# breuner/elbencho

Hardware: AMD Instinct MI355X
Metric: seq-read GiB/s into GPU HBM (higher is better)
Workload: dtype raw-bytes; 1 GPU; seqread; model=storage-benchmark seq-read into HBM, threads_per_gpu=16, block_size=4194304, iodepth=1, bench_dir=/dev/shm/elbencho_amd_bench, gpu_staged=True, mmap_zero_copy=True, dynamic_slice=True, verify_on_gpu=True, verify_salt=7, parallelism=single, device=AMD Radeon Graphics, device_numa_node=0

## Files before the change

elbencho_amd/csrc/engine.cpp:

```cpp

#include "engine.h"

#include <fcntl.h>
#include <linux/fs.h>
#include <pthread.h>
#include <sched.h>
#include <sys/ioctl.h>
#include <sys/mman.h>
#include <sys/stat.h>
#include <sys/types.h>
#include <unistd.h>

#include <algorithm>
#include <random>
#include <cerrno>
#include <cstdio>
#include <cstring>

#include "netbench.h"
#include "uring.h"

namespace eb {

static constexpr uint64_t INTERRUPT_CHECK_INTERVAL = 128;
// ... 898 lines not shown

    const uint64_t mapBPF = (cfg.random || cfg.strided) ? (fileSize / bs) : numBlocksPerFile;
    const uint64_t virtFileLen = mapBPF * bs;

    const bool dynamic = cfg.dynamicSlice && !cfg.random && !cfg.strided &&
                         !cfg.backward && cfg.numThreads == cfg.numDataSetThreads;

    std::unique_ptr<OffsetGen> gen;
    if (dynamic) {
    } else if (cfg.random || cfg.strided) {
        uint64_t numBlocksTotal = mapBPF * numFiles;
        uint64_t rangeLen = bs * (numBlocksTotal / cfg.numDataSetThreads);
        uint64_t rangeOff = (uint64_t)globalRank * rangeLen;
        if (cfg.strided) {
            gen = std::make_unique<OffsetGenStrided>(bs, globalRank, cfg.numDataSetThreads);
            gen->reset(0, bs * numBlocksTotal);
        } else {
            gen = makeOffsetGen(rangeOff, rangeLen);
        }
    } else {
        uint64_t myStart, myLen;
        fairShareSlice(virtFileLen * numFiles, myStart, myLen);
        if (!myLen) return;
        gen = makeOffsetGen(myStart, myLen);
    }

    const int nSlots = (int)hostBufs.size();
    constexpr uint64_t VERIFY_FETCH_INTERVAL = 64;
    uint64_t sinceFetch = 0;
    BlockSpec spec;
    uint64_t opCount = 0;
    int slot = 0;

    auto fetchVerify = [&]() {
        GpuVerifyResult r = gpu->fetchVerifyResult();
        if (r.numMismatches)
            throw WorkerError("Data verification failed (GPU). First bad file offset: " +
                              std::to_string(r.firstBadFileOffset) +
                              "; mismatching 8-byte words: " +
                              std::to_string(r.numMismatches));
    };

    if (doVerify && !isWrite) (void)gpu->fetchVerifyResult();

    const uint64_t totalBlocks = numBlocksPerFile * numFiles;

    auto nextBlock = [&](uint64_t& fileIdx, uint64_t& inFileOff,
                         uint64_t& ioLen) -> bool {
        if (dynamic) {
            for (;;) {
                uint64_t b = eng.dynCursor.fetch_add(1, std::memory_order_relaxed);
                if (b >= totalBlocks) return false;
                fileIdx = b / numBlocksPerFile;
                inFileOff = (b % numBlocksPerFile) * bs;
                if (inFileOff >= fileSize) continue;
                ioLen = std::min(bs, fileSize - inFileOff);
                return true;
            }
        }
        while (gen->next(spec)) {
            if (!virtFileLen) return false;
            fileIdx = spec.offset / virtFileLen;
            if (fileIdx >= numFiles) continue;
            inFileOff = spec.offset - fileIdx * virtFileLen;
            if (inFileOff >= fileSize) continue;
            ioLen = std::min(spec.len, fileSize - inFileOff);
            return true;
        }
        return false;
    };

    uint64_t fileIdx, inFileOff, ioLen;
    while (nextBlock(fileIdx, inFileOff, ioLen)) {
        if ((opCount++ % INTERRUPT_CHECK_INTERVAL) == 0) checkInterrupt();

        rateLimiter.wait(ioLen);

        if (lat && gpu->timedPairActive(slot))
            addIoLat(gpu->timedElapsedUSec(slot));

        if (isWrite) {
            preWriteFill(slot, ioLen, inFileOff);
            if (lat) gpu->recordTimedStart(slot);
            gpu->copyToHostAsync(slot, bases[fileIdx] + inFileOff, ioLen);
            if (lat) gpu->recordTimedEnd(slot);
        } else {
            if (lat) gpu->recordTimedStart(slot);
            gpu->copyFromHostAsync(slot, bases[fileIdx] + inFileOff, ioLen);
            if (lat) gpu->recordTimedEnd(slot);
            if (doVerify && (inFileOff % 8 == 0) && (ioLen % 16 == 0)) {
                gpu->verifyChecksumDevAsync(slot, ioLen, inFileOff,
                                            (uint64_t)cfg.verifySalt);
                if (++sinceFetch >= VERIFY_FETCH_INTERVAL) {
                    fetchVerify();
                    sinceFetch = 0;
                }
            } else if (doVerify) {
                uint64_t bad = verifyChecksumCPU(bases[fileIdx] + inFileOff, ioLen,
                                                 inFileOff, (uint64_t)cfg.verifySalt);
                if (bad != UINT64_MAX)
                    throw WorkerError("Data verification failed. First bad file offset: " +
                                      std::to_string(bad));
            }
        }

        liveOps.bytes.fetch_add(ioLen, std::memory_order_relaxed);
        liveOps.iops.fetch_add(1, std::memory_order_relaxed);
        slot = (slot + 1) % nSlots;

        if ((opCount & 127) == 0) gpu->syncStream();
    }

    gpu->syncStream();
    if (lat)
        for (int s = 0; s < nSlots; s++)
            if (gpu->timedPairActive(s)) addIoLat(gpu->timedElapsedUSec(s));
    if (doVerify && !isWrite) fetchVerify();
}

void Worker::fileModeBlocksUring(bool isWrite)
{
    const auto& cfg = eng.cfg;
    const uint64_t fileSize = eng.effFileSize;
    const uint64_t bs = cfg.blockSize;
    const size_t numFiles = cfg.paths.size();
    const uint64_t numBlocksPerFile = (fileSize + bs - 1) / bs;
    const int depth = cfg.ioDepth;
    const bool lat = cfg.measureLat;

    const bool rwMixActive = isWrite && (cfg.rwMixPct > 0 || isDedicatedReader);

    FdGuard fg;
    int rwFlags = isWrite ? ((cfg.verifyDirect || rwMixActive) ? O_RDWR : O_WRONLY) : O_RDONLY;
    int openFlags = rwFlags | (cfg.directIO ? O_DIRECT : 0);
    if (isWrite && cfg.pathType == PathType::FILE) openFlags |= O_CREAT;
    for (const auto& p : cfg.paths) {
        int fd = open(p.c_str(), openFlags, 0644);
        if (fd < 0) throwErrno("open", p);
        fg.fds.push_back(fd);
        if (isWrite && cfg.pathType == PathType::FILE) {
            if (cfg.truncate && ftruncate(fd, 0)) throwErrno("truncate", p);
            if (cfg.truncToSize != UINT64_MAX && ftruncate(fd, fileSize))
                throwErrno("truncate-to-size", p);
            if (cfg.preallocFile && fallocate(fd, 0, 0, fileSize)) throwErrno("fallocate", p);
        }
        applyFadvise(fd, cfg.fadviseFlags, p);
    }

    const uint64_t mapBPF = (cfg.random || cfg.strided) ? (fileSize / bs) : numBlocksPerFile;
    const uint64_t virtFileLen = mapBPF * bs;
// ... 1858 lines not shown
```

elbencho_amd/csrc/gpu.h:

```cpp

#pragma once

#include <cstdint>
#include <string>
#include <vector>

#include "crc.h"

namespace eb {

struct GpuVerifyResult {
    uint64_t numMismatches;
    uint64_t firstBadFileOffset;
};

void gpuHostRegister(void* ptr, uint64_t len);
bool gpuHostRegisterTry(void* ptr, uint64_t len);
void gpuHostUnregister(void* ptr);

class GpuCtx;

int gpuDeviceCount();

double gpuVerifyBenchGBs(uint64_t len, int iters, bool lds, int dev);

uint64_t gpuCrcTileBytes();
uint64_t gpuCrcWaveBytes();

std::string gpuProbeError();

std::string gpuDeviceName(int deviceId);

int gpuNumaNode(int deviceId);

class GpuCtx {
public:
    GpuCtx(int deviceId, int numSlots, uint64_t bufSize, bool pinnedHostBufs);
    ~GpuCtx();
    GpuCtx(const GpuCtx&) = delete;
    GpuCtx& operator=(const GpuCtx&) = delete;

    int deviceId() const { return devId; }
    char* hostBuf(int slot) const;
    uint64_t bufSize() const { return slotSize; }
    int numSlots() const { return slots; }
    uint64_t slotStride() const;

    void snapshotSlots(std::vector<char>& dst);

    void bindThread();

    void copyFromHostAsync(int slot, const void* src, uint64_t len);
    void copyToHostAsync(int slot, void* dst, uint64_t len);
    void copyH2DAsync(int slot, uint64_t len);
    void copyH2DRangeAsync(int firstSlot, int count);
    void copyD2HAsync(int slot, uint64_t len);
    void syncStream();

    void recordSlotEvent(int slot);
    void waitSlotEvent(int slot);

    void recordTimedStart(int slot);
    void recordTimedEnd(int slot);
    bool timedPairActive(int slot) const;
    uint64_t timedElapsedUSec(int slot);

    void verifyChecksumDevAsync(int slot, uint64_t len, uint64_t fileOff, uint64_t salt,
                                bool ldsVariant = false);
    GpuVerifyResult fetchVerifyResult();


    void fillRandDev(int slot, uint64_t len, uint64_t seed, bool fastAlgo = false);

    void fillChecksumDev(int slot, uint64_t len, uint64_t fileOff, uint64_t salt);

    GpuVerifyResult verifyChecksumDev(int slot, uint64_t len, uint64_t fileOff, uint64_t salt,
                                      bool ldsVariant = false);

    void blockVarRefillDev(int slot, uint64_t len, uint64_t refillLen, uint64_t seed,
                           bool fastAlgo = false);


    void crcDevAsync(int slot, uint64_t len, CrcAlgo algo, uint64_t partialBase);

    uint32_t crcFetch(CrcAlgo algo, uint64_t totalLen, uint64_t tileCount);

    uint32_t crcDev(int slot, uint64_t len, CrcAlgo algo);

private:
    struct Impl;
    Impl* impl;
    int devId;
    uint64_t slotSize;
    int slots;
};

}
```

elbencho_amd/csrc/gpu_kernels.hip:

```cpp

#include <hip/hip_runtime.h>

#include <cstdio>
#include <map>
#include <mutex>
#include <stdexcept>
#include <string>
#include <vector>

#include "crc.h"
#include "gpu.h"

namespace eb {

#define HIP_CHECK(cmd)                                                                 \
    do {                                                                               \
        hipError_t e = (cmd);                                                          \
        if (e != hipSuccess)                                                           \
            throw std::runtime_error(std::string("HIP error: ") + hipGetErrorString(e) \
                                     + " at " __FILE__ ":" + std::to_string(__LINE__)); \
    } while (0)


__device__ __forceinline__ uint64_t d_splitmix64(uint64_t& state)
{
    uint64_t z = (state += 0x9E3779B97F4A7C15ULL);
    z = (z ^ (z >> 30)) * 0xBF58476D1CE4E5B9ULL;
    z = (z ^ (z >> 27)) * 0x94D049BB133111EBULL;
    return z ^ (z >> 31);
}

__device__ __forceinline__ uint64_t d_rotl64(uint64_t x, int k)
{
    return (x << k) | (x >> (64 - k));
}
// ... 141 lines not shown
        uint64_t exp0 = off0 + salt;
        uint64_t exp1 = off0 + 8 + salt;
        if (v.x != exp0) {
            localBad++;
            if (off0 < localFirst) localFirst = off0;
        }
        if (v.y != exp1) {
            localBad++;
            if (off0 + 8 < localFirst) localFirst = off0 + 8;
        }
    }

    if (tid == 0 && (n64 & 1)) {
        uint64_t offT = fileOff + (n64 - 1) * 8;
        if (((const uint64_t*)buf)[n64 - 1] != offT + salt) {
            localBad++;
            if (offT < localFirst) localFirst = offT;
        }
    }

#pragma unroll
    for (int delta = 32; delta > 0; delta >>= 1) {
        localBad += __shfl_down(localBad, delta, 64);
        unsigned long long other = __shfl_down(localFirst, delta, 64);
        if (other < localFirst) localFirst = other;
    }

    if ((threadIdx.x & 63) == 0 && localBad) {
        atomicAdd(&out[0], localBad);
        atomicMin(&out[1], localFirst);
    }
}

__global__ __launch_bounds__(256) void ebVerifyChecksumLdsKernel(
    const ulonglong2* __restrict__ buf, uint64_t n64, uint64_t fileOff,
    uint64_t salt, unsigned long long* __restrict__ out)
{
    const uint64_t nVec2 = n64 / 2;
    constexpr int VPT = 4;
    __shared__ ulonglong2 lds[256 * VPT];
    __shared__ unsigned long long blkBad, blkFirst;
    if (threadIdx.x == 0) {
        blkBad = 0;
        blkFirst = ~0ULL;
    }
    __syncthreads();

    unsigned long long localBad = 0, localFirst = ~0ULL;
    const uint64_t tileElems = (uint64_t)blockDim.x * VPT;

    for (uint64_t tileBase = (uint64_t)blockIdx.x * tileElems; tileBase < nVec2;
         tileBase += (uint64_t)gridDim.x * tileElems) {
#pragma unroll
        for (int v = 0; v < VPT; v++) {
            uint64_t idx = tileBase + (uint64_t)v * blockDim.x + threadIdx.x;
            if (idx < nVec2) lds[v * blockDim.x + threadIdx.x] = buf[idx];
        }
        __syncthreads();
#pragma unroll
        for (int v = 0; v < VPT; v++) {
            uint64_t idx = tileBase + (uint64_t)v * blockDim.x + threadIdx.x;
            if (idx >= nVec2) continue;
            ulonglong2 val = lds[v * blockDim.x + threadIdx.x];
            uint64_t off0 = fileOff + idx * 16;
            if (val.x != off0 + salt) {
                localBad++;
// ... 201 lines not shown
static hipStream_t sharedStream(int devId, int& poolSizeOut)
{
    static std::mutex mtx;
    static std::map<int, std::vector<hipStream_t>> pools;
    static std::map<int, int> next;
    static const int poolSize = [] {
        const char* v = getenv("EB_GPU_SHARED_STREAMS");
        int n = v ? atoi(v) : 8;
        return (n >= 1 && n <= 64) ? n : 0;
    }();

    poolSizeOut = poolSize;
    if (!poolSize) return nullptr;

    std::lock_guard<std::mutex> lk(mtx);
    auto& pool = pools[devId];
    if (pool.empty()) {
        pool.resize(poolSize);
        for (int i = 0; i < poolSize; i++)
            HIP_CHECK(hipStreamCreateWithFlags(&pool[i], hipStreamNonBlocking));
    }
    return pool[next[devId]++ % poolSize];
}

struct GpuCtx::Impl {
    hipStream_t stream = nullptr;
    bool ownStream = true;
    char* devBase = nullptr;
    char* hostBase = nullptr;
    uint64_t slotStride = 0;
    std::vector<char*> devBufs;
    std::vector<char*> hostBufs;
    std::vector<hipEvent_t> slotEvents;
    std::vector<hipEvent_t> timedStart, timedEnd;
    std::vector<char> timedActive;
    bool hostPinned = false;
    unsigned long long* verifyOutDev = nullptr;
    unsigned long long* verifyOutHost = nullptr;
    uint64_t fillCallCounter = 0;
    bool verifyDirty = false;

    uint32_t* crcTabDev[2] = {nullptr, nullptr};
    CrcShift crcTileShift[2];
    uint32_t* crcPartDev = nullptr;
    uint32_t* crcPartHost = nullptr;
    uint64_t crcPartCap = 0;
    struct CrcCall { uint64_t base, len; };
    std::vector<CrcCall> crcPending;
};

GpuCtx::GpuCtx(int deviceId, int numSlots, uint64_t bufSize, bool pinnedHostBufs)
    : impl(new Impl), devId(deviceId), slotSize(bufSize), slots(numSlots)
{
    HIP_CHECK(hipSetDevice(deviceId));
    int poolSize = 0;
    hipStream_t shared = sharedStream(deviceId, poolSize);
    if (shared) {
        impl->stream = shared;
        impl->ownStream = false;
    } else {
        HIP_CHECK(hipStreamCreateWithFlags(&impl->stream, hipStreamNonBlocking));
    }

    impl->hostPinned = pinnedHostBufs;
    impl->devBufs.resize(numSlots, nullptr);
    impl->hostBufs.resize(numSlots, nullptr);

    impl->slotStride = (bufSize + 4095) & ~4095ULL;
    HIP_CHECK(hipMalloc(&impl->devBase, impl->slotStride * numSlots));
    if (pinnedHostBufs) {
        static const unsigned hostFlags = [] {
            const char* v = getenv("EB_GPU_HOSTALLOC");
            return (v && v[0] == 'n') ? hipHostMallocNonCoherent : hipHostMallocDefault;
        }();
        HIP_CHECK(hipHostMalloc(&impl->hostBase, impl->slotStride * numSlots, hostFlags));
    } else {
        if (posix_memalign((void**)&impl->hostBase, 4096, impl->slotStride * numSlots))
            throw std::runtime_error("host buffer alloc failed");
    }
    for (int i = 0; i < numSlots; i++) {
        impl->devBufs[i] = impl->devBase + (uint64_t)i * impl->slotStride;
        impl->hostBufs[i] = impl->hostBase + (uint64_t)i * impl->slotStride;
    }

    impl->slotEvents.resize(numSlots, nullptr);
    static const bool evBlock = [] {
        const char* v = getenv("EB_GPU_EVBLOCK");
        return v && v[0] == '1';
    }();
    unsigned evFlags = hipEventDisableTiming | (evBlock ? hipEventBlockingSync : 0);
    for (int i = 0; i < numSlots; i++)
        HIP_CHECK(hipEventCreateWithFlags(&impl->slotEvents[i], evFlags));

    HIP_CHECK(hipMalloc(&impl->verifyOutDev, 2 * sizeof(unsigned long long)));
    HIP_CHECK(hipHostMalloc(&impl->verifyOutHost, 2 * sizeof(unsigned long long),
                            hipHostMallocDefault));

    impl->verifyOutHost[0] = 0;
    impl->verifyOutHost[1] = ~0ULL;
    HIP_CHECK(hipMemcpy(impl->verifyOutDev, impl->verifyOutHost,
                        2 * sizeof(unsigned long long), hipMemcpyHostToDevice));
}

GpuCtx::~GpuCtx()
{
    (void)hipSetDevice(devId);
    if (impl->devBase) (void)hipFree(impl->devBase);
    if (impl->hostBase) {
        if (impl->hostPinned)
            (void)hipHostFree(impl->hostBase);
        else
            free(impl->hostBase);
    }
    for (auto e : impl->slotEvents)
        if (e) (void)hipEventDestroy(e);
    for (auto e : impl->timedStart)
        if (e) (void)hipEventDestroy(e);
    for (auto e : impl->timedEnd)
        if (e) (void)hipEventDestroy(e);
    if (impl->verifyOutDev) (void)hipFree(impl->verifyOutDev);
    if (impl->verifyOutHost) (void)hipHostFree(impl->verifyOutHost);
    for (auto p : impl->crcTabDev)
        if (p) (void)hipFree(p);
    if (impl->crcPartDev) (void)hipFree(impl->crcPartDev);
    if (impl->crcPartHost) (void)hipHostFree(impl->crcPartHost);
    if (impl->stream && impl->ownStream) (void)hipStreamDestroy(impl->stream);
    delete impl;
}

char* GpuCtx::hostBuf(int slot) const { return impl->hostBufs[slot]; }

void GpuCtx::bindThread() { HIP_CHECK(hipSetDevice(devId)); }

uint64_t GpuCtx::slotStride() const { return impl->slotStride; }

void GpuCtx::snapshotSlots(std::vector<char>& dst)
{
    dst.resize(impl->slotStride * (uint64_t)slots);
    if (dst.empty()) return;
    HIP_CHECK(hipMemcpyAsync(dst.data(), impl->devBase, dst.size(), hipMemcpyDeviceToHost,
                             impl->stream));
    HIP_CHECK(hipStreamSynchronize(impl->stream));
}

void GpuCtx::copyFromHostAsync(int slot, const void* src, uint64_t len)
{
    HIP_CHECK(hipMemcpyAsync(impl->devBufs[slot], src, len, hipMemcpyHostToDevice,
                             impl->stream));
}

void GpuCtx::copyToHostAsync(int slot, void* dst, uint64_t len)
{
    HIP_CHECK(hipMemcpyAsync(dst, impl->devBufs[slot], len, hipMemcpyDeviceToHost,
                             impl->stream));
// ... 65 lines not shown
    return (uint64_t)(ms * 1000.0f);
}

static void requireAligned(const char* what, uint64_t len, uint64_t lenAlign,
                           uint64_t fileOff = 0)
{
    if (len % lenAlign)
        throw std::invalid_argument(std::string(what) + ": len " + std::to_string(len) +
                                    " is not a multiple of " + std::to_string(lenAlign));
    if (fileOff % 8)
        throw std::invalid_argument(std::string(what) + ": fileOff " +
                                    std::to_string(fileOff) + " is not a multiple of 8");
}

void GpuCtx::verifyChecksumDevAsync(int slot, uint64_t len, uint64_t fileOff, uint64_t salt,
                                    bool ldsVariant)
{
    requireAligned("verifyChecksumDev", len, 8, fileOff);
    uint64_t n64 = len / 8;
    if (!n64) return;
    dim3 grid = gridForBytes(n64 / 2);
    if (ldsVariant)
        hipLaunchKernelGGL(ebVerifyChecksumLdsKernel, grid, dim3(256), 0, impl->stream,
                           (const ulonglong2*)impl->devBufs[slot], n64, fileOff, salt,
                           impl->verifyOutDev);
    else
        hipLaunchKernelGGL(ebVerifyChecksumKernel, grid, dim3(256), 0, impl->stream,
                           (const ulonglong2*)impl->devBufs[slot], n64, fileOff, salt,
                           impl->verifyOutDev);
    HIP_CHECK(hipGetLastError());
    impl->verifyDirty = true;
}

GpuVerifyResult GpuCtx::fetchVerifyResult()
{
    if (!impl->verifyDirty) return GpuVerifyResult{0, ~0ULL};
    HIP_CHECK(hipMemcpyAsync(impl->verifyOutHost, impl->verifyOutDev,
                             2 * sizeof(unsigned long long), hipMemcpyDeviceToHost,
                             impl->stream));
    HIP_CHECK(hipStreamSynchronize(impl->stream));
    GpuVerifyResult r{impl->verifyOutHost[0], impl->verifyOutHost[1]};
    impl->verifyOutHost[0] = 0;
    impl->verifyOutHost[1] = ~0ULL;
    HIP_CHECK(hipMemcpyAsync(impl->verifyOutDev, impl->verifyOutHost,
                             2 * sizeof(unsigned long long), hipMemcpyHostToDevice,
                             impl->stream));
    HIP_CHECK(hipStreamSynchronize(impl->stream));
    impl->verifyDirty = false;
    return r;
}

void GpuCtx::fillRandDev(int slot, uint64_t len, uint64_t seed, bool fastAlgo)
{
    requireAligned("fillRandDev", len, 16);
    uint64_t nVec2 = len / 16;
    uint64_t seq = ++impl->fillCallCounter;
    if (nVec2) {
        if (fastAlgo) {
            dim3 grid = gridForBytes(nVec2);
            hipLaunchKernelGGL(ebFillFastKernel, grid, dim3(256), 0, impl->stream,
                               (ulonglong2*)impl->devBufs[slot], nVec2,
                               seed + seq * 0x9E3779B9ULL);
        } else {
            dim3 grid = gridForBytes(nVec2 / (FILL_U64S_PER_STEP / 2));
            hipLaunchKernelGGL(ebFillRandKernel, grid, dim3(256), 0, impl->stream,
                               (ulonglong2*)impl->devBufs[slot], nVec2,
                               seed + seq * 0x9E3779B9ULL);
        }
        HIP_CHECK(hipGetLastError());
    }
}

void GpuCtx::fillChecksumDev(int slot, uint64_t len, uint64_t fileOff, uint64_t salt)
{
    requireAligned("fillChecksumDev", len, 8, fileOff);
    uint64_t n64 = len / 8;
    if (!n64) return;
    dim3 grid = gridForBytes(n64);
    hipLaunchKernelGGL(ebFillChecksumKernel, grid, dim3(256), 0, impl->stream,
                       (uint64_t*)impl->devBufs[slot], n64, fileOff, salt);
    HIP_CHECK(hipGetLastError());
}

GpuVerifyResult GpuCtx::verifyChecksumDev(int slot, uint64_t len, uint64_t fileOff, uint64_t salt,
// ... 139 lines not shown

    auto launch = [&] {
        if (lds)
            hipLaunchKernelGGL(ebVerifyChecksumLdsKernel, grid, dim3(256), 0, s,
                               buf, n64, 0, 7, out);
        else
            hipLaunchKernelGGL(ebVerifyChecksumKernel, grid, dim3(256), 0, s,
                               buf, n64, 0, 7, out);
    };

    launch();
    launch();
    HIP_CHECK(hipStreamSynchronize(s));

    hipEvent_t e0, e1;
    HIP_CHECK(hipEventCreate(&e0));
    HIP_CHECK(hipEventCreate(&e1));
    HIP_CHECK(hipEventRecord(e0, s));
    for (int i = 0; i < iters; i++) launch();
    HIP_CHECK(hipEventRecord(e1, s));
    HIP_CHECK(hipEventSynchronize(e1));
    float ms = 0;
    HIP_CHECK(hipEventElapsedTime(&ms, e0, e1));

    (void)hipEventDestroy(e0);
    (void)hipEventDestroy(e1);
    (void)hipStreamDestroy(s);
    (void)hipFree(buf);
    (void)hipFree(out);

    return (double)len * iters / (ms / 1000.0) / 1e9;
}

}
```

elbencho_amd/csrc/module.cpp:

```cpp

#include <pybind11/pybind11.h>
#include <pybind11/stl.h>

#include <execinfo.h>
#include <csignal>
#include <cstdio>
#include <cstdlib>
#include <cstring>
#include <mutex>
#include <optional>
#include <unistd.h>

#include <fcntl.h>

#include "crc.h"
#include "engine.h"
#include "httpdata.h"
#include "s3srv.h"
#include "gpu.h"
#include "histogram.h"

namespace py = pybind11;
using namespace eb;

namespace {

EngineConfig configFromDict(const py::dict& d)
{
    EngineConfig c;

    auto getU64 = [&](const char* k, uint64_t def) -> uint64_t {
        return d.contains(k) ? d[k].cast<uint64_t>() : def;
    };
    auto getI = [&](const char* k, int64_t def) -> int64_t {
        return d.contains(k) ? d[k].cast<int64_t>() : def;
    };
    auto getB = [&](const char* k, bool def) -> bool {
        return d.contains(k) ? d[k].cast<bool>() : def;
    };
    auto getS = [&](const char* k, std::string def) -> std::string {
        return d.contains(k) ? d[k].cast<std::string>() : def;
    };

    if (d.contains("paths")) c.paths = d["paths"].cast<std::vector<std::string>>();
    std::string pt = getS("path_type", "file");
    c.pathType = (pt == "dir") ? PathType::DIR : (pt == "bdev") ? PathType::BLOCKDEV
// ... 37 lines not shown
        c.treeDirs = d["tree_dirs"].cast<std::vector<std::string>>();
    if (d.contains("tree_files"))
        c.treeFiles = d["tree_files"].cast<std::vector<std::pair<std::string, uint64_t>>>();
    c.shareSize = getU64("sharesize", 0);
    c.treeRoundRobin = getB("tree_round_robin", false);
    c.treeRandomize = getB("tree_rand", false);
    c.netbenchIsServer = getB("netbench_is_server", false);
    if (d.contains("netbench_servers"))
        c.netbenchServers = d["netbench_servers"].cast<std::vector<std::string>>();
    c.netbenchPort = (int)getI("netbench_port", 2611);
    c.netbenchNumConns = (int)getI("netbench_num_conns", 0);
    c.respSize = getU64("resp_size", 1);
    c.sendBufSize = (int)getI("send_buf", 0);
    c.recvBufSize = (int)getI("recv_buf", 0);
    if (d.contains("netdevs"))
        c.netDevs = d["netdevs"].cast<std::vector<std::string>>();
    c.blockVarPct = (int)getI("blockvar_pct", 100);
    c.blockVarAlgo = getS("blockvar_algo", "fast");
    c.randAlgo = getS("rand_algo", "balanced_single");
    if (d.contains("gpu_ids")) c.gpuIDs = d["gpu_ids"].cast<std::vector<int>>();
    c.gpuPinnedHostBufs = getB("gpu_pinned", true);
    c.measureLat = getB("lat", false);
    c.limitReadBps = getU64("limit_read_bps", 0);
    c.limitWriteBps = getU64("limit_write_bps", 0);
    c.ignoreDelErrors = getB("ignore_del_errors", false);
    c.dirSharing = getB("dir_sharing", false);
    c.infiniteLoop = getB("inf_loop", false);
    c.dynamicSlice = getB("dynamic_slice", false);
    c.benchSeed = getU64("bench_seed", 0x243F6A8885A308D3ULL);

    return c;
}

py::dict resultToDict(const WorkerResult& r)
{
    py::dict d;
    d["rank"] = r.rank;
    d["elapsed_usec"] = r.elapsedUSec;
    d["entries"] = r.total.entries;
    d["bytes"] = r.total.bytes;
    d["iops"] = r.total.iops;
    d["stonewall_entries"] = r.stonewall.entries;
    d["stonewall_bytes"] = r.stonewall.bytes;
    d["stonewall_iops"] = r.stonewall.iops;
    d["stonewall_elapsed_usec"] = r.stonewallElapsedUSec;
    d["rm_entries"] = r.totalReadMix.entries;
    d["rm_bytes"] = r.totalReadMix.bytes;
    d["rm_iops"] = r.totalReadMix.iops;
    d["rm_stonewall_entries"] = r.stonewallReadMix.entries;
    d["rm_stonewall_bytes"] = r.stonewallReadMix.bytes;
    d["rm_stonewall_iops"] = r.stonewallReadMix.iops;
    d["io_lat"] = r.ioLatVec;
    d["entry_lat"] = r.entryLatVec;
    d["io_lat_rm"] = r.ioLatReadMixVec;
    d["entry_lat_rm"] = r.entryLatReadMixVec;
    d["error"] = r.error;
    return d;
}

extern "C" void ebFaultHandler(int sig)
{
    void* frames[64];
    int n = backtrace(frames, 64);

    const char* name = (sig == SIGSEGV)   ? "SIGSEGV (segmentation fault)"
                       : (sig == SIGFPE)  ? "SIGFPE (floating point exception)"
                       : (sig == SIGBUS)  ? "SIGBUS (bus error; can be caused by a "
                                            "truncated mmap'ed file)"
                       : (sig == SIGILL)  ? "SIGILL (illegal instruction)"
                       : (sig == SIGABRT) ? "SIGABRT (abort)"
                                          : "fatal signal";
    dprintf(STDERR_FILENO, "\nelbencho-amd: caught %s — native backtrace:\n", name);
    backtrace_symbols_fd(frames, n, STDERR_FILENO);

    const char* tmpdir = getenv("TMPDIR");
    char path[256];
    snprintf(path, sizeof(path), "%s/elbencho_amd_fault_trace.txt",
             tmpdir ? tmpdir : "/tmp");
    int fd = open(path, O_WRONLY | O_CREAT | O_APPEND, 0644);
    if (fd >= 0) {
        dprintf(fd, "caught %s — native backtrace:\n", name);
        backtrace_symbols_fd(frames, n, fd);
        close(fd);
        dprintf(STDERR_FILENO, "(trace also appended to %s)\n", path);
    }

    signal(sig, SIG_DFL);
    raise(sig);
// ... 198 lines not shown
            std::memcpy(ctx.hostBuf(0), thenBuf.data(), thenBuf.size());
            ctx.copyH2DAsync(0, thenBuf.size());
            ctx.syncStream();
            push(ctx.verifyChecksumDev(0, thenBuf.size(), then->second, salt, lds));
        }
        return out;
    }, py::arg("items"), py::arg("salt"), py::arg("lds") = false,
       py::arg("then") = py::none(), py::arg("dev") = 0);

    m.def("gpu_crc", [](py::bytes data, const std::string& algo, int dev, uint64_t guard,
                        int sentinel) {
        CrcAlgo a = crcAlgoFromName(algo);
        std::string buf = data;
        py::gil_scoped_release rel;
        const uint64_t total = buf.size() + guard;
        GpuCtx ctx(dev, 1, std::max<uint64_t>(total, 16), true);
        std::memcpy(ctx.hostBuf(0), buf.data(), buf.size());
        std::memset(ctx.hostBuf(0) + buf.size(), sentinel, guard);
        if (total) ctx.copyH2DAsync(0, total);
        ctx.syncStream();
        return ctx.crcDev(0, buf.size(), a);
    }, py::arg("data"), py::arg("algo"), py::arg("dev") = 0, py::arg("guard") = 0,
       py::arg("sentinel") = 0);
    m.def("gpu_crc_tile_bytes", &gpuCrcTileBytes);
    m.def("gpu_crc_wave_bytes", &gpuCrcWaveBytes);

    m.def("gpu_verify_bench",
          [](uint64_t len, int iters, bool lds, int dev) {
              py::gil_scoped_release rel;
              return gpuVerifyBenchGBs(len, iters, lds, dev);
          },
          py::arg("len"), py::arg("iters") = 50, py::arg("lds") = false,
          py::arg("dev") = 0);

    m.def("gpu_fill_rand", [](uint64_t len, uint64_t seed, int dev, bool fast) {
        GpuCtx ctx(dev, 1, len, true);
        ctx.fillRandDev(0, len, seed, fast);
        ctx.copyD2HAsync(0, len);
        ctx.syncStream();
        return py::bytes(ctx.hostBuf(0), len);
    }, py::arg("len"), py::arg("seed"), py::arg("dev") = 0, py::arg("fast") = false);

    m.def("gpu_blockvar_refill", [](uint64_t len, uint64_t refillLen, uint64_t seed,
                                    int dev, bool fast) {
        GpuCtx ctx(dev, 1, len, true);
        std::memset(ctx.hostBuf(0), 0, len);
        ctx.copyH2DAsync(0, len);
        ctx.syncStream();
        ctx.blockVarRefillDev(0, len, refillLen, seed, fast);
        ctx.copyD2HAsync(0, len);
        ctx.syncStream();
        return py::bytes(ctx.hostBuf(0), len);
    }, py::arg("len"), py::arg("refill_len"), py::arg("seed"), py::arg("dev") = 0,
       py::arg("fast") = false);

    m.def("gpu_kernel_bench", [](uint64_t len, int iters, int dev) {
        GpuCtx ctx(dev, 1, len, true);
        auto timeIt = [&](auto&& fn) {
            fn();
            ctx.syncStream();
            auto t0 = std::chrono::steady_clock::now();
            for (int i = 0; i < iters; i++) fn();
            ctx.syncStream();
            auto dt = std::chrono::duration<double>(std::chrono::steady_clock::now() - t0)
                          .count();
            return (double)len * iters / dt / 1e9;
// ... 205 lines not shown
```

Measured before the change: 52.09 GiB/s.

## Batch GPU checksum verification into one kernel launch per slot group

Verification requests for up to eight slots are collected and checked by a single batched kernel that splits its grid across the buffers, replacing one launch per block. The fetch path resets the counters with a device-to-device copy from a preset buffer and waits once on an event, where it used to do two stream syncs with a host round-trip. The final drain skips the extra stream sync when the fetch already waited. Also adds an H2D link probe, a batch-test binding and a cached empty histogram list. The cost is delayed verification granularity and a capped grid per batch that may reduce per-buffer parallelism.

After: 52.13 GiB/s (median of 2 runs). No clear change (+0.1%).

```diff
diff --git a/elbencho_amd/csrc/engine.cpp b/elbencho_amd/csrc/engine.cpp
--- a/elbencho_amd/csrc/engine.cpp
+++ b/elbencho_amd/csrc/engine.cpp
@@ -954,13 +954,21 @@
     uint64_t opCount = 0;
     int slot = 0;
 
-    auto fetchVerify = [&]() {
-        GpuVerifyResult r = gpu->fetchVerifyResult();
+    auto raiseVerify = [](const GpuVerifyResult& r) {
         if (r.numMismatches)
             throw WorkerError("Data verification failed (GPU). First bad file offset: " +
                               std::to_string(r.firstBadFileOffset) +
                               "; mismatching 8-byte words: " +
                               std::to_string(r.numMismatches));
+    };
+
+    GpuVerifyItem vBatch[VERIFY_BATCH_MAX];
+    int vBatchLen = 0;
+    const int vBatchMax = std::min(nSlots, (int)VERIFY_BATCH_MAX);
+    auto flushVerify = [&]() {
+        if (!vBatchLen) return;
+        gpu->verifyChecksumBatchDevAsync(vBatch, vBatchLen, (uint64_t)cfg.verifySalt);
+        vBatchLen = 0;
     };
 
     if (doVerify && !isWrite) (void)gpu->fetchVerifyResult();
@@ -1011,13 +1019,16 @@
             gpu->copyFromHostAsync(slot, bases[fileIdx] + inFileOff, ioLen);
             if (lat) gpu->recordTimedEnd(slot);
             if (doVerify && (inFileOff % 8 == 0) && (ioLen % 16 == 0)) {
-                gpu->verifyChecksumDevAsync(slot, ioLen, inFileOff,
-                                            (uint64_t)cfg.verifySalt);
+                vBatch[vBatchLen++] = GpuVerifyItem{slot, ioLen, inFileOff};
                 if (++sinceFetch >= VERIFY_FETCH_INTERVAL) {
-                    fetchVerify();
+                    flushVerify();
+                    raiseVerify(gpu->fetchVerifyResult());
                     sinceFetch = 0;
+                } else if (vBatchLen >= vBatchMax) {
+                    flushVerify();
                 }
             } else if (doVerify) {
+                flushVerify();
                 uint64_t bad = verifyChecksumCPU(bases[fileIdx] + inFileOff, ioLen,
                                                  inFileOff, (uint64_t)cfg.verifySalt);
                 if (bad != UINT64_MAX)
@@ -1033,11 +1044,17 @@
         if ((opCount & 127) == 0) gpu->syncStream();
     }
 
-    gpu->syncStream();
+    GpuVerifyResult finalVerify{0, UINT64_MAX};
+    bool waited = false;
+    if (doVerify && !isWrite) {
+        flushVerify();
+        finalVerify = gpu->fetchVerifyResult(&waited);
+    }
+    if (!waited) gpu->syncStream();
     if (lat)
         for (int s = 0; s < nSlots; s++)
             if (gpu->timedPairActive(s)) addIoLat(gpu->timedElapsedUSec(s));
-    if (doVerify && !isWrite) fetchVerify();
+    raiseVerify(finalVerify);
 }
 
 void Worker::fileModeBlocksUring(bool isWrite)
diff --git a/elbencho_amd/csrc/gpu.h b/elbencho_amd/csrc/gpu.h
--- a/elbencho_amd/csrc/gpu.h
+++ b/elbencho_amd/csrc/gpu.h
@@ -23,6 +23,17 @@
 int gpuDeviceCount();
 
 double gpuVerifyBenchGBs(uint64_t len, int iters, bool lds, int dev);
+
+double gpuH2DLinkProbeGBs(void* hostBase, uint64_t hostLen, uint64_t blockSize, int numStreams,
+                          int passes, int dev);
+
+constexpr int VERIFY_BATCH_MAX = 8;
+
+struct GpuVerifyItem {
+    int slot;
+    uint64_t len;
+    uint64_t fileOff;
+};
 
 uint64_t gpuCrcTileBytes();
 uint64_t gpuCrcWaveBytes();
@@ -67,7 +78,8 @@
 
     void verifyChecksumDevAsync(int slot, uint64_t len, uint64_t fileOff, uint64_t salt,
                                 bool ldsVariant = false);
-    GpuVerifyResult fetchVerifyResult();
+    void verifyChecksumBatchDevAsync(const GpuVerifyItem* items, int count, uint64_t salt);
+    GpuVerifyResult fetchVerifyResult(bool* waited = nullptr);
 
 
     void fillRandDev(int slot, uint64_t len, uint64_t seed, bool fastAlgo = false);
diff --git a/elbencho_amd/csrc/gpu_kernels.hip b/elbencho_amd/csrc/gpu_kernels.hip
--- a/elbencho_amd/csrc/gpu_kernels.hip
+++ b/elbencho_amd/csrc/gpu_kernels.hip
@@ -1,6 +1,8 @@
 
 #include <hip/hip_runtime.h>
 
+#include <algorithm>
+#include <chrono>
 #include <cstdio>
 #include <map>
 #include <mutex>
@@ -208,6 +210,75 @@
     }
 }
 
+struct VerifyBatchArgs {
+    const ulonglong2* buf[VERIFY_BATCH_MAX];
+    uint64_t n64[VERIFY_BATCH_MAX];
+    uint64_t fileOff[VERIFY_BATCH_MAX];
+    uint32_t blockEnd[VERIFY_BATCH_MAX];
+    uint32_t count;
+};
+
+__global__ __launch_bounds__(256) void ebVerifyChecksumBatchKernel(
+    const VerifyBatchArgs args, uint64_t salt, unsigned long long* __restrict__ out)
+{
+    const ulonglong2* __restrict__ buf = args.buf[0];
+    uint64_t n64 = args.n64[0];
+    uint64_t fileOff = args.fileOff[0];
+    uint32_t firstBlock = 0, endBlock = args.blockEnd[0];
+#pragma unroll
+    for (uint32_t i = 1; i < VERIFY_BATCH_MAX; i++)
+        if (i < args.count && blockIdx.x >= args.blockEnd[i - 1]) {
+            buf = args.buf[i];
+            n64 = args.n64[i];
+            fileOff = args.fileOff[i];
+            firstBlock = args.blockEnd[i - 1];
+            endBlock = args.blockEnd[i];
+        }
+    if (blockIdx.x >= endBlock) return;
+
+    uint64_t tid = (uint64_t)(blockIdx.x - firstBlock) * blockDim.x + threadIdx.x;
+    uint64_t stride = (uint64_t)(endBlock - firstBlock) * blockDim.x;
+    uint64_t nVec2 = n64 / 2;
+
+    unsigned long long localBad = 0;
+    unsigned long long localFirst = ~0ULL;
+
+    for (uint64_t i = tid; i < nVec2; i += stride) {
+        ulonglong2 v = buf[i];
+        uint64_t off0 = fileOff + i * 16;
+        uint64_t exp0 = off0 + salt;
+        uint64_t exp1 = off0 + 8 + salt;
+        if (v.x != exp0) {
+            localBad++;
+            if (off0 < localFirst) localFirst = off0;
+        }
+        if (v.y != exp1) {
+            localBad++;
+            if (off0 + 8 < localFirst) localFirst = off0 + 8;
+        }
+    }
+
+    if (tid == 0 && (n64 & 1)) {
+        uint64_t offT = fileOff + (n64 - 1) * 8;
+        if (((const uint64_t*)buf)[n64 - 1] != offT + salt) {
+            localBad++;
+            if (offT < localFirst) localFirst = offT;
+        }
+    }
+
+#pragma unroll
+    for (int delta = 32; delta > 0; delta >>= 1) {
+        localBad += __shfl_down(localBad, delta, 64);
+        unsigned long long other = __shfl_down(localFirst, delta, 64);
+        if (other < localFirst) localFirst = other;
+    }
+
+    if ((threadIdx.x & 63) == 0 && localBad) {
+        atomicAdd(&out[0], localBad);
+        atomicMin(&out[1], localFirst);
+    }
+}
+
 __global__ __launch_bounds__(256) void ebVerifyChecksumLdsKernel(
     const ulonglong2* __restrict__ buf, uint64_t n64, uint64_t fileOff,
     uint64_t salt, unsigned long long* __restrict__ out)
@@ -480,6 +551,8 @@
     bool hostPinned = false;
     unsigned long long* verifyOutDev = nullptr;
     unsigned long long* verifyOutHost = nullptr;
+    unsigned long long* verifyResetDev = nullptr;
+    hipEvent_t fetchEvent = nullptr;
     uint64_t fillCallCounter = 0;
     bool verifyDirty = false;
 
@@ -543,6 +616,10 @@
     impl->verifyOutHost[1] = ~0ULL;
     HIP_CHECK(hipMemcpy(impl->verifyOutDev, impl->verifyOutHost,
                         2 * sizeof(unsigned long long), hipMemcpyHostToDevice));
+    HIP_CHECK(hipMalloc(&impl->verifyResetDev, 2 * sizeof(unsigned long long)));
+    HIP_CHECK(hipMemcpy(impl->verifyResetDev, impl->verifyOutHost,
+                        2 * sizeof(unsigned long long), hipMemcpyHostToDevice));
+    HIP_CHECK(hipEventCreateWithFlags(&impl->fetchEvent, evFlags));
 }
 
 GpuCtx::~GpuCtx()
@@ -563,6 +640,8 @@
         if (e) (void)hipEventDestroy(e);
     if (impl->verifyOutDev) (void)hipFree(impl->verifyOutDev);
     if (impl->verifyOutHost) (void)hipHostFree(impl->verifyOutHost);
+    if (impl->verifyResetDev) (void)hipFree(impl->verifyResetDev);
+    if (impl->fetchEvent) (void)hipEventDestroy(impl->fetchEvent);
     for (auto p : impl->crcTabDev)
         if (p) (void)hipFree(p);
     if (impl->crcPartDev) (void)hipFree(impl->crcPartDev);
@@ -694,22 +773,61 @@
     impl->verifyDirty = true;
 }
 
-GpuVerifyResult GpuCtx::fetchVerifyResult()
-{
+void GpuCtx::verifyChecksumBatchDevAsync(const GpuVerifyItem* items, int count, uint64_t salt)
+{
+    if (count < 0 || count > VERIFY_BATCH_MAX)
+        throw std::invalid_argument("verifyChecksumBatchDev: " + std::to_string(count) +
+                                    " items, the limit is " +
+                                    std::to_string(VERIFY_BATCH_MAX));
+    VerifyBatchArgs args = {};
+    uint64_t want[VERIFY_BATCH_MAX];
+    uint64_t wantSum = 0;
+    uint32_t n = 0;
+    for (int i = 0; i < count; i++) {
+        const GpuVerifyItem& it = items[i];
+        requireAligned("verifyChecksumBatchDev", it.len, 8, it.fileOff);
+        if (it.slot < 0 || it.slot >= slots || it.len > impl->slotStride)
+            throw std::invalid_argument("verifyChecksumBatchDev: item " + std::to_string(i) +
+                                        " lies outside the slot ring");
+        if (!it.len) continue;
+        args.buf[n] = (const ulonglong2*)impl->devBufs[it.slot];
+        args.n64[n] = it.len / 8;
+        args.fileOff[n] = it.fileOff;
+        want[n] = gridForBytes(it.len / 16).x;
+        wantSum += want[n];
+        n++;
+    }
+    if (!n) return;
+
+    constexpr uint64_t GRID_CAP = 4096;
+    uint32_t end = 0;
+    for (uint32_t i = 0; i < n; i++) {
+        uint64_t blocks = (wantSum > GRID_CAP) ? want[i] * GRID_CAP / wantSum : want[i];
+        end += (uint32_t)std::max<uint64_t>(blocks, 1);
+        args.blockEnd[i] = end;
+    }
+    args.count = n;
+
+    hipLaunchKernelGGL(ebVerifyChecksumBatchKernel, dim3(end), dim3(256), 0, impl->stream,
+                       args, salt, impl->verifyOutDev);
+    HIP_CHECK(hipGetLastError());
+    impl->verifyDirty = true;
+}
+
+GpuVerifyResult GpuCtx::fetchVerifyResult(bool* waited)
+{
+    if (waited) *waited = impl->verifyDirty;
     if (!impl->verifyDirty) return GpuVerifyResult{0, ~0ULL};
     HIP_CHECK(hipMemcpyAsync(impl->verifyOutHost, impl->verifyOutDev,
                              2 * sizeof(unsigned long long), hipMemcpyDeviceToHost,
                              impl->stream));
-    HIP_CHECK(hipStreamSynchronize(impl->stream));
-    GpuVerifyResult r{impl->verifyOutHost[0], impl->verifyOutHost[1]};
-    impl->verifyOutHost[0] = 0;
-    impl->verifyOutHost[1] = ~0ULL;
-    HIP_CHECK(hipMemcpyAsync(impl->verifyOutDev, impl->verifyOutHost,
-                             2 * sizeof(unsigned long long), hipMemcpyHostToDevice,
+    HIP_CHECK(hipMemcpyAsync(impl->verifyOutDev, impl->verifyResetDev,
+                             2 * sizeof(unsigned long long), hipMemcpyDeviceToDevice,
                              impl->stream));
-    HIP_CHECK(hipStreamSynchronize(impl->stream));
+    HIP_CHECK(hipEventRecord(impl->fetchEvent, impl->stream));
+    HIP_CHECK(hipEventSynchronize(impl->fetchEvent));
     impl->verifyDirty = false;
-    return r;
+    return GpuVerifyResult{impl->verifyOutHost[0], impl->verifyOutHost[1]};
 }
 
 void GpuCtx::fillRandDev(int slot, uint64_t len, uint64_t seed, bool fastAlgo)
@@ -917,4 +1035,52 @@
     return (double)len * iters / (ms / 1000.0) / 1e9;
 }
 
-}
+double gpuH2DLinkProbeGBs(void* hostBase, uint64_t hostLen, uint64_t blockSize, int numStreams,
+                          int passes, int dev)
+{
+    if (!blockSize || hostLen < blockSize || numStreams < 1 || numStreams > 16 || passes < 1)
+        throw std::invalid_argument("gpuH2DLinkProbeGBs: bad geometry");
+    HIP_CHECK(hipSetDevice(dev));
+    HIP_CHECK(hipHostRegister(hostBase, hostLen, hipHostRegisterDefault));
+
+    std::vector<hipStream_t> streams(numStreams, nullptr);
+    std::vector<char*> devBufs(numStreams, nullptr);
+    double gbs = 0;
+    try {
+        for (int s = 0; s < numStreams; s++) {
+            HIP_CHECK(hipStreamCreateWithFlags(&streams[s], hipStreamNonBlocking));
+            HIP_CHECK(hipMalloc(&devBufs[s], blockSize));
+        }
+        const uint64_t numBlocks = hostLen / blockSize;
+        auto onePass = [&] {
+            for (uint64_t b = 0; b < numBlocks; b++) {
+                int s = (int)(b % numStreams);
+                HIP_CHECK(hipMemcpyAsync(devBufs[s], (char*)hostBase + b * blockSize, blockSize,
+                                         hipMemcpyHostToDevice, streams[s]));
+            }
+        };
+        auto drain = [&] {
+            for (auto s : streams) HIP_CHECK(hipStreamSynchronize(s));
+        };
+        onePass();
+        drain();
+        auto t0 = std::chrono::steady_clock::now();
+        for (int p = 0; p < passes; p++) onePass();
+        drain();
+        double dt = std::chrono::duration<double>(std::chrono::steady_clock::now() - t0).count();
+        gbs = (double)numBlocks * blockSize * passes / dt / 1e9;
+    } catch (...) {
+        for (auto s : streams)
+            if (s) (void)hipStreamDestroy(s);
+        for (auto p : devBufs)
+            if (p) (void)hipFree(p);
+        (void)hipHostUnregister(hostBase);
+        throw;
+    }
+    for (auto s : streams) (void)hipStreamDestroy(s);
+    for (auto p : devBufs) (void)hipFree(p);
+    (void)hipHostUnregister(hostBase);
+    return gbs;
+}
+
+}
diff --git a/elbencho_amd/csrc/module.cpp b/elbencho_amd/csrc/module.cpp
--- a/elbencho_amd/csrc/module.cpp
+++ b/elbencho_amd/csrc/module.cpp
@@ -12,6 +12,7 @@
 #include <unistd.h>
 
 #include <fcntl.h>
+#include <sys/mman.h>
 
 #include "crc.h"
 #include "engine.h"
@@ -115,6 +116,16 @@
     return c;
 }
 
+py::object histVecToList(const std::vector<uint64_t>& v)
+{
+    static const std::vector<uint64_t> emptyVec = LatencyHistogram().toVec();
+    if (v == emptyVec) {
+        static py::object* emptyList = new py::object(py::cast(emptyVec));
+        return *emptyList;
+    }
+    return py::cast(v);
+}
+
 py::dict resultToDict(const WorkerResult& r)
 {
     py::dict d;
@@ -133,10 +144,10 @@
     d["rm_stonewall_entries"] = r.stonewallReadMix.entries;
     d["rm_stonewall_bytes"] = r.stonewallReadMix.bytes;
     d["rm_stonewall_iops"] = r.stonewallReadMix.iops;
-    d["io_lat"] = r.ioLatVec;
-    d["entry_lat"] = r.entryLatVec;
-    d["io_lat_rm"] = r.ioLatReadMixVec;
-    d["entry_lat_rm"] = r.entryLatReadMixVec;
+    d["io_lat"] = histVecToList(r.ioLatVec);
+    d["entry_lat"] = histVecToList(r.entryLatVec);
+    d["io_lat_rm"] = histVecToList(r.ioLatReadMixVec);
+    d["entry_lat_rm"] = histVecToList(r.entryLatReadMixVec);
     d["error"] = r.error;
     return d;
 }
@@ -401,6 +412,74 @@
           },
           py::arg("len"), py::arg("iters") = 50, py::arg("lds") = false,
           py::arg("dev") = 0);
+
+    m.def("gpu_h2d_link_probe",
+          [](const std::string& path, uint64_t blockSize, int streams, int passes, int dev) {
+              py::gil_scoped_release rel;
+              int fd = open(path.c_str(), O_RDONLY);
+              if (fd < 0) throw std::runtime_error("gpu_h2d_link_probe: cannot open " + path);
+              off_t len = lseek(fd, 0, SEEK_END);
+              void* p = len > 0 ? mmap(nullptr, (size_t)len, PROT_READ,
+                                       MAP_SHARED | MAP_POPULATE, fd, 0)
+                                : MAP_FAILED;
+              close(fd);
+              if (p == MAP_FAILED)
+                  throw std::runtime_error("gpu_h2d_link_probe: cannot map " + path);
+              double gbs;
+              try {
+                  gbs = gpuH2DLinkProbeGBs(p, (uint64_t)len, blockSize, streams, passes, dev);
+              } catch (...) {
+                  munmap(p, (size_t)len);
+                  throw;
+              }
+              munmap(p, (size_t)len);
+              return gbs;
+          },
+          py::arg("path"), py::arg("block_size") = (uint64_t)4 << 20, py::arg("streams") = 1,
+          py::arg("passes") = 4, py::arg("dev") = 0);
+
+    m.def("gpu_verify_batches",
+          [](const std::vector<std::vector<std::pair<py::bytes, uint64_t>>>& batches,
+             uint64_t salt, int extraFetches, int dev) {
+              std::vector<std::vector<std::string>> bufs;
+              uint64_t maxLen = 16;
+              for (const auto& b : batches) {
+                  if (b.size() > (size_t)VERIFY_BATCH_MAX)
+                      throw std::invalid_argument("gpu_verify_batches: batch too long");
+                  bufs.emplace_back();
+                  for (const auto& it : b) {
+                      bufs.back().emplace_back(it.first);
+                      maxLen = std::max<uint64_t>(maxLen, bufs.back().back().size());
+                  }
+              }
+              std::vector<GpuVerifyResult> res;
+              {
+                  py::gil_scoped_release rel;
+                  GpuCtx ctx(dev, VERIFY_BATCH_MAX, maxLen, true);
+                  for (size_t b = 0; b < bufs.size(); b++) {
+                      GpuVerifyItem items[VERIFY_BATCH_MAX];
+                      for (size_t i = 0; i < bufs[b].size(); i++) {
+                          const std::string& s = bufs[b][i];
+                          std::memcpy(ctx.hostBuf((int)i), s.data(), s.size());
+                          if (!s.empty()) ctx.copyH2DAsync((int)i, s.size());
+                          items[i] = GpuVerifyItem{(int)i, s.size(), batches[b][i].second};
+                      }
+                      ctx.verifyChecksumBatchDevAsync(items, (int)bufs[b].size(), salt);
+                      bool waited = false;
+                      res.push_back(ctx.fetchVerifyResult(&waited));
+                      if (!waited) ctx.syncStream();
+                      for (int e = 0; e < extraFetches; e++)
+                          res.push_back(ctx.fetchVerifyResult());
+                  }
+              }
+              py::list out;
+              for (const auto& r : res)
+                  out.append(py::make_tuple(r.numMismatches, r.firstBadFileOffset));
+              return out;
+          },
+          py::arg("batches"), py::arg("salt"), py::arg("extra_fetches") = 0,
+          py::arg("dev") = 0);
+    m.def("gpu_verify_batch_max", [] { return (int)VERIFY_BATCH_MAX; });
 
     m.def("gpu_fill_rand", [](uint64_t len, uint64_t seed, int dev, bool fast) {
         GpuCtx ctx(dev, 1, len, true);
```

## Replace stream-wide syncs with per-slot events and double-buffered verify windows

Applied to the files above, without the earlier changes.

In the zero-copy read path, the periodic full-stream synchronizations are replaced by per-slot event waits, so a slot is reused only after its previous copy completes. GPU verification results go into two device-side windows that are copied back and reset asynchronously. Each window's result is collected one window later, so the host no longer blocks on a D2H and H2D round trip every 64 blocks. This adds more event bookkeeping and more complex lifetime handling (a quiesce guard and cleanup at destruction), and mismatches are reported later than before.

New measurement: 52.14 GiB/s before, 52.36 GiB/s after (median of 6 runs). No clear change (+0.4%).

```diff
diff --git a/elbencho_amd/csrc/engine.cpp b/elbencho_amd/csrc/engine.cpp
--- a/elbencho_amd/csrc/engine.cpp
+++ b/elbencho_amd/csrc/engine.cpp
@@ -954,8 +954,8 @@
     uint64_t opCount = 0;
     int slot = 0;
 
-    auto fetchVerify = [&]() {
-        GpuVerifyResult r = gpu->fetchVerifyResult();
+    auto collectWindow = [&]() {
+        GpuVerifyResult r = gpu->zcWindowCollect();
         if (r.numMismatches)
             throw WorkerError("Data verification failed (GPU). First bad file offset: " +
                               std::to_string(r.firstBadFileOffset) +
@@ -963,7 +963,23 @@
                               std::to_string(r.numMismatches));
     };
 
-    if (doVerify && !isWrite) (void)gpu->fetchVerifyResult();
+    struct SlotQuiesce {
+        GpuCtx* g;
+        int n;
+        ~SlotQuiesce()
+        {
+            if (!g) return;
+            for (int s = 0; s < n; s++) {
+                try {
+                    if (g->timedPairActive(s)) (void)g->timedElapsedUSec(s);
+                    g->zcWaitSlotCopy(s);
+                } catch (...) {
+                }
+            }
+        }
+    } quiesce{isWrite ? nullptr : gpu.get(), nSlots};
+
+    if (!isWrite) gpu->zcReadBegin();
 
     const uint64_t totalBlocks = numBlocksPerFile * numFiles;
 
@@ -1007,17 +1023,17 @@
             gpu->copyToHostAsync(slot, bases[fileIdx] + inFileOff, ioLen);
             if (lat) gpu->recordTimedEnd(slot);
         } else {
-            if (lat) gpu->recordTimedStart(slot);
-            gpu->copyFromHostAsync(slot, bases[fileIdx] + inFileOff, ioLen);
-            if (lat) gpu->recordTimedEnd(slot);
+            gpu->zcWaitSlotCopy(slot);
+            gpu->zcCopyFromHostAsync(slot, bases[fileIdx] + inFileOff, ioLen, lat);
             if (doVerify && (inFileOff % 8 == 0) && (ioLen % 16 == 0)) {
-                gpu->verifyChecksumDevAsync(slot, ioLen, inFileOff,
-                                            (uint64_t)cfg.verifySalt);
+                gpu->zcVerifyAsync(slot, ioLen, inFileOff, (uint64_t)cfg.verifySalt);
                 if (++sinceFetch >= VERIFY_FETCH_INTERVAL) {
-                    fetchVerify();
+                    collectWindow();
+                    gpu->zcWindowClose();
                     sinceFetch = 0;
                 }
             } else if (doVerify) {
+                collectWindow();
                 uint64_t bad = verifyChecksumCPU(bases[fileIdx] + inFileOff, ioLen,
                                                  inFileOff, (uint64_t)cfg.verifySalt);
                 if (bad != UINT64_MAX)
@@ -1030,14 +1046,18 @@
         liveOps.iops.fetch_add(1, std::memory_order_relaxed);
         slot = (slot + 1) % nSlots;
 
-        if ((opCount & 127) == 0) gpu->syncStream();
-    }
-
-    gpu->syncStream();
-    if (lat)
-        for (int s = 0; s < nSlots; s++)
-            if (gpu->timedPairActive(s)) addIoLat(gpu->timedElapsedUSec(s));
-    if (doVerify && !isWrite) fetchVerify();
+        if (isWrite && (opCount & 127) == 0) gpu->syncStream();
+    }
+
+    if (isWrite) gpu->syncStream();
+    for (int s = 0; s < nSlots; s++) {
+        if (lat && gpu->timedPairActive(s)) addIoLat(gpu->timedElapsedUSec(s));
+        if (!isWrite) gpu->zcWaitSlotCopy(s);
+    }
+    if (doVerify && !isWrite) {
+        collectWindow();
+        if (gpu->zcWindowClose()) collectWindow();
+    }
 }
 
 void Worker::fileModeBlocksUring(bool isWrite)
diff --git a/elbencho_amd/csrc/gpu.h b/elbencho_amd/csrc/gpu.h
--- a/elbencho_amd/csrc/gpu.h
+++ b/elbencho_amd/csrc/gpu.h
@@ -70,6 +70,15 @@
     GpuVerifyResult fetchVerifyResult();
 
 
+    void zcReadBegin();
+    void zcCopyFromHostAsync(int slot, const void* src, uint64_t len, bool timed);
+    void zcWaitSlotCopy(int slot);
+    void zcVerifyAsync(int slot, uint64_t len, uint64_t fileOff, uint64_t salt);
+    bool zcWindowClose();
+    bool zcWindowOutstanding() const;
+    GpuVerifyResult zcWindowCollect();
+
+
     void fillRandDev(int slot, uint64_t len, uint64_t seed, bool fastAlgo = false);
 
     void fillChecksumDev(int slot, uint64_t len, uint64_t fileOff, uint64_t salt);
diff --git a/elbencho_amd/csrc/gpu_kernels.hip b/elbencho_amd/csrc/gpu_kernels.hip
--- a/elbencho_amd/csrc/gpu_kernels.hip
+++ b/elbencho_amd/csrc/gpu_kernels.hip
@@ -475,6 +475,7 @@
     std::vector<char*> devBufs;
     std::vector<char*> hostBufs;
     std::vector<hipEvent_t> slotEvents;
+    unsigned evFlags = 0;
     std::vector<hipEvent_t> timedStart, timedEnd;
     std::vector<char> timedActive;
     bool hostPinned = false;
@@ -482,6 +483,14 @@
     unsigned long long* verifyOutHost = nullptr;
     uint64_t fillCallCounter = 0;
     bool verifyDirty = false;
+
+    std::vector<char> zcCopyPending;
+    unsigned long long* winDev = nullptr;
+    unsigned long long* winHost = nullptr;
+    hipEvent_t winEvent[2] = {nullptr, nullptr};
+    int winCur = 0;
+    int winOutstanding = -1;
+    bool winCurDirty = false;
 
     uint32_t* crcTabDev[2] = {nullptr, nullptr};
     CrcShift crcTileShift[2];
@@ -531,9 +540,9 @@
         const char* v = getenv("EB_GPU_EVBLOCK");
         return v && v[0] == '1';
     }();
-    unsigned evFlags = hipEventDisableTiming | (evBlock ? hipEventBlockingSync : 0);
+    impl->evFlags = hipEventDisableTiming | (evBlock ? hipEventBlockingSync : 0);
     for (int i = 0; i < numSlots; i++)
-        HIP_CHECK(hipEventCreateWithFlags(&impl->slotEvents[i], evFlags));
+        HIP_CHECK(hipEventCreateWithFlags(&impl->slotEvents[i], impl->evFlags));
 
     HIP_CHECK(hipMalloc(&impl->verifyOutDev, 2 * sizeof(unsigned long long)));
     HIP_CHECK(hipHostMalloc(&impl->verifyOutHost, 2 * sizeof(unsigned long long),
@@ -548,6 +557,7 @@
 GpuCtx::~GpuCtx()
 {
     (void)hipSetDevice(devId);
+    if (impl->winDev) (void)hipStreamSynchronize(impl->stream);
     if (impl->devBase) (void)hipFree(impl->devBase);
     if (impl->hostBase) {
         if (impl->hostPinned)
@@ -563,6 +573,10 @@
         if (e) (void)hipEventDestroy(e);
     if (impl->verifyOutDev) (void)hipFree(impl->verifyOutDev);
     if (impl->verifyOutHost) (void)hipHostFree(impl->verifyOutHost);
+    for (auto e : impl->winEvent)
+        if (e) (void)hipEventDestroy(e);
+    if (impl->winDev) (void)hipFree(impl->winDev);
+    if (impl->winHost) (void)hipHostFree(impl->winHost);
     for (auto p : impl->crcTabDev)
         if (p) (void)hipFree(p);
     if (impl->crcPartDev) (void)hipFree(impl->crcPartDev);
@@ -712,6 +726,98 @@
     return r;
 }
 
+
+static constexpr size_t WIN_SET_BYTES = 2 * sizeof(unsigned long long);
+
+void GpuCtx::zcReadBegin()
+{
+    Impl& m = *impl;
+    if (!m.winDev) {
+        m.zcCopyPending.assign(slots, 0);
+        for (int s = 0; s < 2; s++)
+            HIP_CHECK(hipEventCreateWithFlags(&m.winEvent[s], m.evFlags));
+        HIP_CHECK(hipHostMalloc(&m.winHost, 3 * WIN_SET_BYTES, hipHostMallocDefault));
+        for (int s = 0; s < 3; s++) {
+            m.winHost[2 * s] = 0;
+            m.winHost[2 * s + 1] = ~0ULL;
+        }
+        HIP_CHECK(hipMalloc(&m.winDev, 2 * WIN_SET_BYTES));
+        HIP_CHECK(hipMemcpy(m.winDev, m.winHost, 2 * WIN_SET_BYTES, hipMemcpyHostToDevice));
+        return;
+    }
+
+    if (m.winCurDirty || m.winOutstanding >= 0)
+        for (int s = 0; s < 2; s++)
+            HIP_CHECK(hipMemcpyAsync(m.winDev + 2 * s, m.winHost + 4, WIN_SET_BYTES,
+                                     hipMemcpyHostToDevice, m.stream));
+    m.winCur = 0;
+    m.winOutstanding = -1;
+    m.winCurDirty = false;
+}
+
+void GpuCtx::zcCopyFromHostAsync(int slot, const void* src, uint64_t len, bool timed)
+{
+    Impl& m = *impl;
+    if (timed) recordTimedStart(slot);
+    HIP_CHECK(hipMemcpyAsync(m.devBufs[slot], src, len, hipMemcpyHostToDevice, m.stream));
+    if (timed) {
+        recordTimedEnd(slot);
+    } else {
+        HIP_CHECK(hipEventRecord(m.slotEvents[slot], m.stream));
+        m.zcCopyPending[slot] = 1;
+    }
+}
+
+void GpuCtx::zcWaitSlotCopy(int slot)
+{
+    if (impl->zcCopyPending.empty() || !impl->zcCopyPending[slot]) return;
+    HIP_CHECK(hipEventSynchronize(impl->slotEvents[slot]));
+    impl->zcCopyPending[slot] = 0;
+}
+
+void GpuCtx::zcVerifyAsync(int slot, uint64_t len, uint64_t fileOff, uint64_t salt)
+{
+    Impl& m = *impl;
+    requireAligned("verifyChecksumDev", len, 8, fileOff);
+    uint64_t n64 = len / 8;
+    if (!n64) return;
+    hipLaunchKernelGGL(ebVerifyChecksumKernel, gridForBytes(n64 / 2), dim3(256), 0, m.stream,
+                       (const ulonglong2*)m.devBufs[slot], n64, fileOff, salt,
+                       m.winDev + 2 * m.winCur);
+    HIP_CHECK(hipGetLastError());
+    m.winCurDirty = true;
+}
+
+bool GpuCtx::zcWindowClose()
+{
+    Impl& m = *impl;
+    if (!m.winCurDirty) return false;
+    if (m.winOutstanding >= 0)
+        throw std::logic_error("zcWindowClose: the previous window was not collected");
+    const int s = m.winCur;
+    HIP_CHECK(hipMemcpyAsync(m.winHost + 2 * s, m.winDev + 2 * s, WIN_SET_BYTES,
+                             hipMemcpyDeviceToHost, m.stream));
+    HIP_CHECK(hipEventRecord(m.winEvent[s], m.stream));
+    HIP_CHECK(hipMemcpyAsync(m.winDev + 2 * s, m.winHost + 4, WIN_SET_BYTES,
+                             hipMemcpyHostToDevice, m.stream));
+    m.winOutstanding = s;
+    m.winCur = s ^ 1;
+    m.winCurDirty = false;
+    return true;
+}
+
+bool GpuCtx::zcWindowOutstanding() const { return impl->winOutstanding >= 0; }
+
+GpuVerifyResult GpuCtx::zcWindowCollect()
+{
+    Impl& m = *impl;
+    if (m.winOutstanding < 0) return GpuVerifyResult{0, ~0ULL};
+    const int s = m.winOutstanding;
+    HIP_CHECK(hipEventSynchronize(m.winEvent[s]));
+    m.winOutstanding = -1;
+    return GpuVerifyResult{m.winHost[2 * s], m.winHost[2 * s + 1]};
+}
+
 void GpuCtx::fillRandDev(int slot, uint64_t len, uint64_t seed, bool fastAlgo)
 {
     requireAligned("fillRandDev", len, 16);
```
